# FutureSDR/FutureSDR

Hardware: NVIDIA H100
Metric: Msamples/s (higher is better)
Workload: dtype f32

## Files before the change

### futuresdr_b200/csrc/common.cuh

```cuda
#pragma once

#include <cuda_runtime.h>

#include <atomic>
#include <cstdarg>
#include <cstdint>
#include <cstdio>
#include <cstring>
#include <memory>
#include <mutex>
#include <string>
#include <vector>

#include "b200sdr.h"

struct b2s_ctx {
    int device = 0;
    cudaStream_t stream = nullptr;
    bool owns_stream = false;
    cudaStream_t s_h2d = nullptr, s_d2h = nullptr;
    int sm_count = 0;
    size_t smem_optin = 0;
    std::atomic<uint64_t> launches{0};
    std::string err;
    void *ws_dev = nullptr;
    size_t ws_bytes = 0;
    cudaEvent_t hev[16] = {};
    bool hev_ready = false;
    std::mutex host_mu;
    unsigned *d_status = nullptr;
    uint64_t flag_ops = 0;
    std::atomic<uint64_t> bytes_held{0};
};

struct PerDeviceOnce {
    std::atomic<uint64_t> mask{0};
    bool need(int dev) const { return ((mask.load(std::memory_order_acquire) >> (dev & 63)) & 1ull) == 0; }
    void done(int dev) { mask.fetch_or(1ull << (dev & 63), std::memory_order_release); }
};

#ifdef __CUDACC__
__device__ __forceinline__ void mac(float &acc, float x, float t) { acc = fmaf(x, t, acc); }
__device__ __forceinline__ void mac(float2 &acc, float2 x, float t) {
    acc.x = fmaf(x.x, t, acc.x);
    acc.y = fmaf(x.y, t, acc.y);
}
__device__ __forceinline__ void mac(float2 &acc, float2 x, float2 t) {
    acc.x = fmaf(x.x, t.x, acc.x);
    acc.x = fmaf(-x.y, t.y, acc.x);
    acc.y = fmaf(x.x, t.y, acc.y);
    acc.y = fmaf(x.y, t.x, acc.y);
}

template <typename S> __device__ __forceinline__ S zero_of();
template <> __device__ __forceinline__ float zero_of<float>() { return 0.0f; }
template <> __device__ __forceinline__ float2 zero_of<float2>() { return make_float2(0.f, 0.f); }

namespace cp_async {
__device__ __forceinline__ void ca4(float *dst_smem, const float *src) {
    const unsigned d = (unsigned)__cvta_generic_to_shared(dst_smem);
    asm volatile("cp.async.ca.shared.global [%0], [%1], 4;" ::"r"(d), "l"(src) : "memory");
}
__device__ __forceinline__ void ca4(float *dst_smem, const float *src, bool valid) {
    const unsigned d = (unsigned)__cvta_generic_to_shared(dst_smem);
    asm volatile("cp.async.ca.shared.global [%0], [%1], 4, %2;" ::"r"(d), "l"(src), "r"(valid ? 4 : 0) : "memory");
}
__device__ __forceinline__ void cg16(void *dst_smem, const void *src) {
    const unsigned d = (unsigned)__cvta_generic_to_shared(dst_smem);
    asm volatile("cp.async.cg.shared.global [%0], [%1], 16;" ::"r"(d), "l"(src) : "memory");
}
__device__ __forceinline__ void cg16(void *dst_smem, const void *src, bool valid) {
    const unsigned d = (unsigned)__cvta_generic_to_shared(dst_smem);
    asm volatile("cp.async.cg.shared.global [%0], [%1], 16, %2;" ::"r"(d), "l"(src), "r"(valid ? 16 : 0) : "memory");
}
__device__ __forceinline__ void commit() { asm volatile("cp.async.commit_group;" ::: "memory"); }
template <int N> __device__ __forceinline__ void wait() { asm volatile("cp.async.wait_group %0;" ::"n"(N) : "memory"); }
}
#endif

extern thread_local std::string g_b2s_last_error;

int32_t b2s_fail(b2s_ctx *ctx, int32_t code, const char *fmt, ...);

#define B2S_CUDA(ctx, expr)                                                                   \
    do {                                                                                      \
        cudaError_t e__ = (expr);                                                             \
        if (e__ != cudaSuccess)                                                               \
            return b2s_fail((ctx), B2S_ECUDA, "%s failed: %s (%s:%d)", #expr,                 \
                            cudaGetErrorString(e__), __FILE__, __LINE__);                     \
    } while (0)

#define B2S_CHECK_LAUNCH(ctx)                                                                 \
    do {                                                                                      \
        (ctx)->launches.fetch_add(1, std::memory_order_relaxed);                              \
        B2S_CUDA((ctx), cudaGetLastError());                                                  \
    } while (0)

struct DeviceGuard {
    int prev = -1;
    explicit DeviceGuard(int dev) {
        cudaGetDevice(&prev);
        if (prev != dev) cudaSetDevice(dev);
        else prev = -1;
    }
    ~DeviceGuard() {
        if (prev >= 0) cudaSetDevice(prev);
    }
};

#define B2S_TRY(expr)                                                                         \
    do {                                                                                      \
        const int32_t rc__ = (expr);                                                          \
        if (rc__ != B2S_OK) return rc__;                                                      \
    } while (0)

template <auto K>
int32_t smem_optin(b2s_ctx *ctx, size_t bytes, int threads = 0, int *resident = nullptr) {
    static PerDeviceOnce optin;
    static std::atomic<int> ctas[64];
    if (bytes > 48 * 1024 && optin.need(ctx->device)) {
        B2S_CUDA(ctx, cudaFuncSetAttribute(K, cudaFuncAttributeMaxDynamicSharedMemorySize, (int)bytes));
        optin.done(ctx->device);
    }
    if (resident) {
        std::atomic<int> &n = ctas[ctx->device & 63];
        int r = n.load(std::memory_order_relaxed);
        if (!r) {
            if (cudaOccupancyMaxActiveBlocksPerMultiprocessor(&r, K, threads, bytes) != cudaSuccess || r < 1) { cudaGetLastError(); r = 1; }
            n.store(r, std::memory_order_relaxed);
        }
        *resident = r;
    }
    return B2S_OK;
}

enum class Mem { Device, Pinned };

template <typename T, Mem M = Mem::Device>
class Buf {
  public:
    Buf() = default;
    Buf(Buf &&o) noexcept { swap(o); }
    Buf &operator=(Buf &&o) noexcept {
        Buf(std::move(o)).swap(*this);
        return *this;
    }
    ~Buf() { reset(); }

    T *get() const { return p_; }
    size_t size() const { return n_; }
    explicit operator bool() const { return p_ != nullptr; }

    void reset() {
        if (!ctx_) return;
        if (M == Mem::Device) cudaFree(p_);
        else cudaFreeHost(p_);
        ctx_->bytes_held -= n_ * sizeof(T);
        ctx_ = nullptr; p_ = nullptr; n_ = 0;
    }
    int32_t alloc(b2s_ctx *ctx, size_t n, const char *what) {
        reset();
        void *p = nullptr;
        const cudaError_t e = M == Mem::Device ? cudaMalloc(&p, n * sizeof(T))
                                               : cudaHostAlloc(&p, n * sizeof(T), cudaHostAllocDefault);
        if (e != cudaSuccess) {
            cudaGetLastError();
            return b2s_fail(ctx, B2S_ENOMEM, "%s: %zu bytes: %s", what, n * sizeof(T), cudaGetErrorString(e));
        }
        ctx_ = ctx; p_ = static_cast<T *>(p); n_ = n;
        ctx->bytes_held += n * sizeof(T);
        return B2S_OK;
    }
    int32_t upload(b2s_ctx *ctx, const T *host, size_t n, const char *what) {
        B2S_TRY(alloc(ctx, n, what));
        B2S_CUDA(ctx, cudaMemcpyAsync(p_, host, n * sizeof(T), cudaMemcpyHostToDevice, ctx->stream));
        return B2S_OK;
    }
    int32_t reserve(b2s_ctx *ctx, size_t n, const char *what) {
        if (n_ >= n) return B2S_OK;
        B2S_CUDA(ctx, cudaStreamSynchronize(ctx->stream));
        return alloc(ctx, n, what);
    }

  private:
    void swap(Buf &o) noexcept {
        std::swap(ctx_, o.ctx_); std::swap(p_, o.p_); std::swap(n_, o.n_);
    }
    b2s_ctx *ctx_ = nullptr;
    T *p_ = nullptr;
    size_t n_ = 0;
};

template <typename P> struct PlanDeleter {
    void operator()(P *p) const {
        if (!p) return;
        DeviceGuard g(p->ctx->device);
        cudaStreamSynchronize(p->ctx->stream);
        delete p;
    }
};
template <typename P> using PlanPtr = std::unique_ptr<P, PlanDeleter<P>>;

void nvtx_push(const char *name);
void nvtx_pop();
struct NvtxRange { explicit NvtxRange(const char *n) { nvtx_push(n); } ~NvtxRange() { nvtx_pop(); } };
int32_t peer_flag_set_launch(b2s_ctx *ctx, unsigned *flag, unsigned value, cudaStream_t st);
int32_t peer_flag_wait_launch(b2s_ctx *ctx, const unsigned *flag, unsigned value, cudaStream_t st);

static inline size_t sat_sub(size_t a, size_t b) { return a > b ? a - b : 0; }
static inline size_t ceil_div(size_t a, size_t b) { return (a + b - 1) / b; }
static inline size_t round_up(size_t a, size_t b) { return ceil_div(a, b) * b; }

static inline bool overlap(const void *p, size_t pb, const void *q, size_t qb) {
    const uintptr_t a = (uintptr_t)p, b = (uintptr_t)q;
    return pb && qb && a < b + qb && b < a + pb;
}
static inline bool bad_alias(const void *out, size_t ob, size_t oi, const void *in, size_t ib, size_t ii) {
    if (!overlap(out, ob, in, ib)) return false;
    return !(out == in && oi == ii);
}
static inline bool word_aligned(const void *p) { return ((uintptr_t)p & 3) == 0; }

static inline size_t kind_in_bytes(b2s_kind k) { return k == B2S_F32_F32 ? 4 : 8; }
static inline size_t kind_tap_floats(b2s_kind k) { return k == B2S_C32_C32 ? 2 : 1; }
```

### futuresdr_b200/csrc/pfbarb.cu

```cuda
#include <cmath>
#include <cstdlib>

#include "pfb_common.cuh"

namespace {
constexpr int kSB = 32;
constexpr int kPaThreads = 256;
constexpr int kDescCap = 4096;
constexpr int kPaSmemMax = 3 * kDescCap * 4 + 2 * 64 * 1024;

struct SubRec {
    uint32_t out0;
    float tau;
    float mu;
    uint32_t base_flag;
};
}

struct b2s_pfbarb {
    b2s_ctx *ctx = nullptr;
    size_t num_filters = 0, T = 0, ntaps = 0;
    float rate = 1.f, delay = 1.f;
    Buf<float2> d_arms;
    PfbWindows win;
    float tau = 0.f, bf = 0.f, mu = 0.f;
    size_t base_index = 0;
    bool boundary = false;
    bool periodic = false;
    uint64_t lambda = 0, out_per_period = 0, gpos = 0;
    std::vector<SubRec> tab;
    Buf<SubRec> d_tab;
    Buf<SubRec, Mem::Pinned> h_recs;
    Buf<SubRec> d_recs;
};

namespace {

__host__ __device__ __forceinline__ uint32_t pfb_arm_index(float bf) {
    const float f = floorf(bf);
    return f > 0.f ? (f < 4294967296.f ? (uint32_t)f : 0xffffffffu) : 0u;
}

inline size_t pfbarb_per_sample_max(float rate, size_t num_filters) {
    if (rate <= (float)num_filters) return (size_t)std::ceil(rate) + 1;
    return (size_t)std::ceil((double)rate * (1.0 + 1.0 / (double)num_filters)) + 2;
}

__device__ __forceinline__ float2 pfb_x(const float2 *__restrict__ hist, const float2 *__restrict__ in, int L,
                                        long long idx) {
    return idx < L ? hist[idx] : __ldg(in + (idx - L));
}

struct PaParams {
    const float2 *in, *hist;
    float2 *out;
    const float2 *arms;
    const SubRec *recs;
    long long n_in, nsub, nout;
    int sub_per_cta, N, T, sb_len;
    float delay;
    int arms_in_smem, tile_in_smem, tile_cap;
    int periodic;
    unsigned long long lambda, out_per_period, R, g0, lsb_first;
    long long O_g0;
};

struct SubStart { float tau, mu; uint32_t base_flag; long long s_beg, s_end, o_start; };

__device__ __forceinline__ SubStart pfb_sub_start(const PaParams &P, long long i) {
    SubStart r;
    if (P.periodic) {
        const unsigned long long lsb = P.lsb_first + (unsigned long long)i;
        const unsigned long long k = lsb / P.R, j = lsb - k * P.R;
        const SubRec rec = P.recs[j];
        const unsigned long long gs = k * P.lambda + j * (unsigned long long)P.sb_len;
        const unsigned long long ge = min(gs + (unsigned long long)P.sb_len, (k + 1) * P.lambda);
        r.tau = rec.tau; r.mu = rec.mu; r.base_flag = rec.base_flag;
        r.s_beg = (long long)gs - (long long)P.g0;
        r.s_end = min((long long)ge - (long long)P.g0, P.n_in);
        r.o_start = (long long)(k * P.out_per_period + rec.out0) - P.O_g0;
    } else {
        const SubRec rec = P.recs[i];
        r.tau = rec.tau; r.mu = rec.mu; r.base_flag = rec.base_flag;
        r.s_beg = i * P.sb_len;
        r.s_end = min(r.s_beg + P.sb_len, P.n_in);
        r.o_start = rec.out0;
    }
    return r;
}

__global__ void __launch_bounds__(kPaThreads) pfb_kernel(const PaParams P) {
    extern __shared__ __align__(16) unsigned char psm[];
    uint32_t *d_s1 = reinterpret_cast<uint32_t *>(psm);
    uint32_t *d_b0 = d_s1 + kDescCap;
    float *d_mu = reinterpret_cast<float *>(d_b0 + kDescCap);
    float2 *s_x = reinterpret_cast<float2 *>(d_mu + kDescCap);
    float2 *s_arms = s_x + (P.tile_in_smem ? P.tile_cap : 0);
    const int N = P.N, T = P.T;

    const long long sb0 = (long long)blockIdx.x * P.sub_per_cta;
    const long long sb1 = min(sb0 + P.sub_per_cta, P.nsub);
    const SubStart first = pfb_sub_start(P, sb0);
    const long long o_first = max(first.o_start, 0ll);
    const long long o_end = sb1 == P.nsub ? P.nout : pfb_sub_start(P, sb1).o_start;
    const long long s_lo = max(first.s_beg, 0ll);
    const long long s_hi = pfb_sub_start(P, sb1 - 1).s_end;
    const int TS = P.arms_in_smem ? (T | 1) : T;
    float *s_tap = reinterpret_cast<float *>(s_arms);
    if (P.arms_in_smem)
        for (int j = threadIdx.x; j < N * T; j += kPaThreads) s_tap[(j / T) * TS + (j % T)] = P.arms[j].x;
    if (P.tile_in_smem) {
        const int cnt = (int)(s_hi - s_lo) + T;
        for (int j = threadIdx.x; j < cnt; j += kPaThreads) s_x[j] = pfb_x(P.hist, P.in, T, s_lo + j);
    }

    for (long long sb = sb0 + threadIdx.x; sb < sb1; sb += kPaThreads) {
        const SubStart r = pfb_sub_start(P, sb);
        float tau = r.tau, mu = r.mu;
        uint32_t base = r.base_flag & 0x7fffffffu;
        bool boundary = (r.base_flag >> 31) != 0;
        long long o = r.o_start - o_first;
        const float fN = (float)N, delay = P.delay;
        for (long long s = r.s_beg; s < r.s_end; s++) {
            while (base < (uint32_t)N) {
                if (boundary) {
                    if (s >= 0) { d_s1[o] = (uint32_t)(s + 1 - s_lo) | 0x80000000u; d_b0[o] = (uint32_t)(N - 1); d_mu[o] = mu; }
                    o++;
                    tau = __fadd_rn(tau, delay);
                    const float bf = __fmul_rn(tau, fN);
                    base = pfb_arm_index(bf);
                    mu = __fsub_rn(bf, (float)base);
                    boundary = false;
                } else if (base == (uint32_t)(N - 1)) {
                    boundary = true;
                    base = (uint32_t)N;
                } else {
                    if (s >= 0) { d_s1[o] = (uint32_t)(s + 1 - s_lo); d_b0[o] = base; d_mu[o] = mu; }
                    o++;
                    tau = __fadd_rn(tau, delay);
                    const float bf = __fmul_rn(tau, fN);
                    base = pfb_arm_index(bf);
                    mu = __fsub_rn(bf, (float)base);
                }
            }
            tau = __fsub_rn(tau, 1.0f);
            base -= (uint32_t)N;
        }
    }
    __syncthreads();

    const float2 *A = P.arms;
    const uint32_t cnt = (uint32_t)(o_end - o_first);
    for (uint32_t o = threadIdx.x; o < cnt; o += kPaThreads) {
        const uint32_t w = d_s1[o];
        const bool boundary = (w >> 31) != 0;
        const int s1 = (int)(w & 0x7fffffffu);
        const uint32_t b0 = d_b0[o];
        const float mu = d_mu[o];
        const float2 *pr = A + (size_t)b0 * T;
        float2 y0 = make_float2(0.f, 0.f), y1 = make_float2(0.f, 0.f);
        if (P.tile_in_smem && P.arms_in_smem) {
            const float *t0 = s_tap + b0 * TS, *t1 = s_tap + (b0 + 1 == (uint32_t)N ? 0u : b0 + 1) * TS;
            const float2 *xb = s_x + s1;
            if (!boundary) {
#pragma unroll 4
                for (int j = 0; j < T; j++) {
                    const float2 v = xb[j];
                    const float ta = t0[j], tb = t1[j];
                    y0.x = fmaf(v.x, ta, y0.x); y0.y = fmaf(v.y, ta, y0.y);
                    y1.x = fmaf(v.x, tb, y1.x); y1.y = fmaf(v.y, tb, y1.y);
                }
            } else {
                const float2 *xa = xb - 1;
                for (int j = 0; j < T; j++) {
                    const float2 va = xa[j], vb = xb[j];
                    const float ta = t0[j], tb = t1[j];
                    y0.x = fmaf(va.x, ta, y0.x); y0.y = fmaf(va.y, ta, y0.y);
                    y1.x = fmaf(vb.x, tb, y1.x); y1.y = fmaf(vb.y, tb, y1.y);
                }
            }
        } else if (P.tile_in_smem) {
            const float2 *xb = s_x + s1;
            if (!boundary) {
#pragma unroll 4
                for (int j = 0; j < T; j++) {
                    const float2 v = xb[j], t = pr[j];
                    y0.x = fmaf(v.x, t.x, y0.x); y0.y = fmaf(v.y, t.x, y0.y);
                    y1.x = fmaf(v.x, t.y, y1.x); y1.y = fmaf(v.y, t.y, y1.y);
                }
            } else {
                const float2 *xa = xb - 1;
                for (int j = 0; j < T; j++) {
                    const float2 va = xa[j], vb = xb[j], t = pr[j];
                    y0.x = fmaf(va.x, t.x, y0.x); y0.y = fmaf(va.y, t.x, y0.y);
                    y1.x = fmaf(vb.x, t.y, y1.x); y1.y = fmaf(vb.y, t.y, y1.y);
                }
            }
        } else {
            const int s0 = boundary ? s1 - 1 : s1;
            for (int j = 0; j < T; j++) {
                const float2 va = pfb_x(P.hist, P.in, T, s_lo + s0 + j), vb = pfb_x(P.hist, P.in, T, s_lo + s1 + j);
                const float2 t = pr[j];
                y0.x = fmaf(va.x, t.x, y0.x); y0.y = fmaf(va.y, t.x, y0.y);
                y1.x = fmaf(vb.x, t.y, y1.x); y1.y = fmaf(vb.y, t.y, y1.y);
            }
        }
        const float a = __fsub_rn(1.0f, mu);
        float2 r;
        r.x = __fadd_rn(__fmul_rn(a, y0.x), __fmul_rn(mu, y1.x));
        r.y = __fadd_rn(__fmul_rn(a, y0.y), __fmul_rn(mu, y1.y));
        P.out[(size_t)o_first + o] = r;
    }
}

struct Timing {
    float tau = 0.f, mu = 0.f;
    uint32_t base = 0;
    bool boundary = false;
    bool operator==(const Timing &o) const { return tau == o.tau && mu == o.mu && base == o.base && boundary == o.boundary; }
    inline uint32_t step(uint32_t N, float fN, float delay) {
        uint32_t o = 0;
        while (base < N) {
            if (boundary) {
                o++;
                tau = tau + delay; const float bf = tau * fN; base = pfb_arm_index(bf); mu = bf - (float)base;
                boundary = false;
            } else if (base == N - 1) {
                boundary = true;
                base = N;
            } else {
                o++;
                tau = tau + delay; const float bf = tau * fN; base = pfb_arm_index(bf); mu = bf - (float)base;
            }
        }
        tau = tau - 1.0f;
        base -= N;
        return o;
    }
    SubRec rec(uint32_t out0) const { return SubRec{out0, tau, mu, base | (boundary ? 0x80000000u : 0u)}; }
};

constexpr int kPerSB = 8;
constexpr uint64_t kMaxPeriod = 1ull << 25;

bool build_periodic_schedule(b2s_pfbarb *p) {
    const uint32_t N = (uint32_t)p->num_filters;
    const float fN = (float)N, delay = p->delay;
    Timing tort, hare;
    uint64_t power = 1, lam = 1;
    hare.step(N, fN, delay);
    while (!(tort == hare)) {
        if (power == lam) {
            if (power > kMaxPeriod) return false;
            tort = hare; power *= 2; lam = 0;
        }
        hare.step(N, fN, delay);
        lam++;
    }
    if (lam > kMaxPeriod) return false;
    const uint64_t R = ceil_div((size_t)lam, (size_t)kPerSB);
    std::vector<SubRec> tab(R);
    Timing t;
    uint64_t o = 0;
    for (uint64_t s = 0; s < lam; s++) {
        if ((s % kPerSB) == 0) tab[s / kPerSB] = t.rec((uint32_t)o);
        o += t.step(N, fN, delay);
        if (o >= (1ull << 32)) return false;
    }
    if (!(t == Timing())) return false;
    p->tab.swap(tab);
    p->lambda = lam; p->out_per_period = o;
    return true;
}

uint64_t outputs_before(const b2s_pfbarb *p, uint64_t c) {
    if (c >= p->lambda) return p->out_per_period + outputs_before(p, c - p->lambda);
    const uint64_t j = c / kPerSB;
    const SubRec &r = p->tab[j];
    Timing t;
    t.tau = r.tau; t.mu = r.mu; t.base = r.base_flag & 0x7fffffffu; t.boundary = (r.base_flag >> 31) != 0;
    uint64_t o = r.out0;
    const uint32_t N = (uint32_t)p->num_filters;
    for (uint64_t s = j * kPerSB; s < c; s++) o += t.step(N, (float)N, p->delay);
    return o;
}

}

extern "C" {

int32_t b2s_pfbarb_period(float rate, size_t num_filters, uint64_t *period_items, uint64_t *outputs_per_period) {
    if (!(rate > 0.f) || num_filters == 0 || !period_items || !outputs_per_period)
        return b2s_fail(nullptr, B2S_EINVAL, "b2s_pfbarb_period: bad argument");
    b2s_pfbarb tmp;
    tmp.num_filters = num_filters; tmp.rate = rate; tmp.delay = 1.0f / rate;
    const bool ok = build_periodic_schedule(&tmp);
    *period_items = ok ? tmp.lambda : 0;
    *outputs_per_period = ok ? tmp.out_per_period : 0;
    return B2S_OK;
}

int32_t b2s_pfbarb_plan_c32(b2s_ctx *ctx, const float *taps, size_t ntaps, size_t num_filters, float rate,
                            b2s_pfbarb **out) {
    if (!ctx || !out || !taps) return b2s_fail(ctx, B2S_EINVAL, "b2s_pfbarb_plan_c32: NULL argument");
    *out = nullptr;
    if (!(rate > 0.f)) return b2s_fail(ctx, B2S_EINVAL, "PfbArbResampler: resampling rate must be greater than zero");
    if (num_filters == 0) return b2s_fail(ctx, B2S_EINVAL, "PfbArbResampler: number of filter banks must be greater than zero");
    if (ntaps < num_filters) return b2s_fail(ctx, B2S_EINVAL, "PfbArbResampler: prototype filter length must be at least num_filters");
    if (num_filters > (1u << 20) || rate > 126.f || pfbarb_per_sample_max(rate, num_filters) * kSB > (size_t)kDescCap)
        return b2s_fail(ctx, B2S_EUNSUPPORTED, "PfbArbResampler: rate %f too large for %zu arms (a sample may produce more outputs than one CTA holds)", (double)rate, num_filters);
    DeviceGuard g(ctx->device);
    PlanPtr<b2s_pfbarb> p(new b2s_pfbarb());
    p->ctx = ctx; p->num_filters = num_filters; p->ntaps = ntaps; p->rate = rate;
    p->delay = 1.0f / rate;
    std::vector<float> arms;
    const size_t T = pfb_partition(taps, ntaps, num_filters, arms);
    p->T = T;
    std::vector<float2> pairs(num_filters * T);
    for (size_t b = 0; b < num_filters; b++)
        for (size_t j = 0; j < T; j++)
            pairs[b * T + j] = make_float2(arms[b * T + T - 1 - j], arms[((b + 1) % num_filters) * T + T - 1 - j]);
    B2S_TRY(p->d_arms.upload(ctx, pairs.data(), pairs.size(), "pfbarb arms"));
    B2S_TRY(p->win.init(ctx, 1, (int)T, false, "pfbarb history"));
    p->periodic = getenv("B2S_PFBARB_NO_PERIODIC") ? false : build_periodic_schedule(p.get());
    if (p->periodic) B2S_TRY(p->d_tab.upload(ctx, p->tab.data(), p->tab.size(), "pfbarb schedule table"));
    B2S_TRY(smem_optin<pfb_kernel>(ctx, kPaSmemMax));
    B2S_CUDA(ctx, cudaStreamSynchronize(ctx->stream));
    B2S_TRY(b2s_pfbarb_reset(p.get()));
    *out = p.release();
    return B2S_OK;
}

void b2s_pfbarb_destroy(b2s_pfbarb *p) { PlanDeleter<b2s_pfbarb>()(p); }

int32_t b2s_pfbarb_reset(b2s_pfbarb *p) {
    if (!p) return b2s_fail(nullptr, B2S_EINVAL, "pfbarb is NULL");
    DeviceGuard g(p->ctx->device);
    p->tau = 0.f; p->bf = 0.f; p->mu = 0.f; p->base_index = 0; p->boundary = false;
    p->gpos = 0;
    return p->win.reset(p->ctx);
}

int32_t b2s_pfbarb_exec(b2s_pfbarb *p, const void *d_in, size_t n_in, void *d_out, size_t n_out_cap,
                        size_t *consumed, size_t *produced, int32_t *call_again) {
    if (!p || !consumed || !produced || !call_again) return b2s_fail(p ? p->ctx : nullptr, B2S_EINVAL, "b2s_pfbarb_exec: NULL argument");
    b2s_ctx *ctx = p->ctx;
    *consumed = 0; *produced = 0; *call_again = 0;
    DeviceGuard g(ctx->device);
    const int T = (int)p->T;
    const float2 *in = (const float2 *)d_in;
    if (!p->win.full()) {
        const size_t c = std::min(p->win.missing(), n_in);
        B2S_TRY(p->win.push(ctx, in, c));
        *consumed = c;
        if (n_in - c > 0) *call_again = 1;
        return B2S_OK;
    }
    const size_t cap = (size_t)((float)n_out_cap / p->rate);
    const size_t n = std::min(n_in, cap);
    if (n == 0) return B2S_OK;
    if (!d_in || !d_out) return b2s_fail(ctx, B2S_EINVAL, "b2s_pfbarb_exec: NULL buffer");
    if (n >= (1ull << 31)) return b2s_fail(ctx, B2S_EUNSUPPORTED, "b2s_pfbarb_exec: more than 2^31 items per call");
    NvtxRange nvtx("b2s_pfbarb_exec");
    PaParams P{};
    P.in = in; P.hist = p->win.hist.get(); P.out = (float2 *)d_out; P.arms = p->d_arms.get();
    P.n_in = (long long)n; P.N = (int)p->num_filters; P.T = T; P.delay = p->delay;
    size_t nout;
    Timing after;
    if (p->periodic) {
        const uint64_t g0 = p->gpos, g1 = g0 + n, lam = p->lambda, R = p->tab.size();
        const uint64_t O0 = outputs_before(p, g0);
        const uint64_t O1 = (g1 / lam) * p->out_per_period + outputs_before(p, g1 % lam);
        nout = (size_t)(O1 - O0);
        if (nout > n_out_cap)
            return b2s_fail(ctx, B2S_ESTATE, "pfbarb: schedule produces %zu > capacity %zu (the reference would overrun its slice)", nout, n_out_cap);
        const uint64_t lsb_first = g0 / kPerSB;
        const uint64_t gl = g1 - 1, lsb_last = (gl / lam) * R + (gl % lam) / kPerSB;
        P.periodic = 1; P.recs = p->d_tab.get(); P.sb_len = kPerSB;
        P.lambda = lam; P.out_per_period = p->out_per_period; P.R = R; P.g0 = g0; P.lsb_first = lsb_first;
        P.O_g0 = (long long)O0;
        P.nsub = (long long)(lsb_last - lsb_first + 1);
    } else {
        const size_t nsub = ceil_div(n, (size_t)kSB);
        B2S_CUDA(ctx, cudaStreamSynchronize(ctx->stream));
        if (std::min(p->d_recs.size(), p->h_recs.size()) < nsub + 1) {
            const size_t want = (nsub + 1) * 5 / 4 + 16;
            B2S_TRY(p->d_recs.reserve(ctx, want, "pfbarb records"));
            B2S_TRY(p->h_recs.reserve(ctx, want, "pfbarb pinned records"));
        }
        Timing t;
        t.tau = p->tau; t.mu = p->mu; t.base = (uint32_t)p->base_index; t.boundary = p->boundary;
        const uint32_t N = (uint32_t)p->num_filters;
        uint64_t o = 0;
        for (size_t s = 0; s < n; s++) {
            if ((s % kSB) == 0) p->h_recs.get()[s / kSB] = t.rec((uint32_t)o);
            o += t.step(N, (float)N, p->delay);
        }
        p->h_recs.get()[nsub] = t.rec((uint32_t)o);
        nout = (size_t)o;
        if (nout > n_out_cap || o >= (1ull << 32))
            return b2s_fail(ctx, B2S_ESTATE, "pfbarb: schedule produces %zu > capacity %zu (the reference would overrun its slice)", nout, n_out_cap);
        after = t;
        B2S_CUDA(ctx, cudaMemcpyAsync(p->d_recs.get(), p->h_recs.get(), (nsub + 1) * sizeof(SubRec), cudaMemcpyHostToDevice, ctx->stream));
        P.periodic = 0; P.recs = p->d_recs.get(); P.sb_len = kSB; P.nsub = (long long)nsub;
    }
    P.nout = (long long)nout;
    const size_t per_sample_max = pfbarb_per_sample_max(p->rate, p->num_filters);
    size_t sub_per_cta = kDescCap / (per_sample_max * P.sb_len);
    if (sub_per_cta == 0) return b2s_fail(ctx, B2S_EUNSUPPORTED, "pfbarb: rate %f too high for the descriptor tile", (double)p->rate);
    sub_per_cta = std::min<size_t>(sub_per_cta, kPaThreads);
    P.sub_per_cta = (int)sub_per_cta;
    const unsigned grid = (unsigned)ceil_div((size_t)P.nsub, sub_per_cta);
    const size_t tile_items = sub_per_cta * P.sb_len + p->T + 2;
    P.tile_in_smem = tile_items * sizeof(float2) <= 64 * 1024;
    P.tile_cap = (int)tile_items;
    const size_t arms_smem_bytes = p->num_filters * (p->T | 1) * sizeof(float);
    P.arms_in_smem = arms_smem_bytes <= 64 * 1024;
    const size_t smem = 3 * kDescCap * sizeof(uint32_t) + (P.tile_in_smem ? tile_items * sizeof(float2) : 0) +
                        (P.arms_in_smem ? arms_smem_bytes : 0);
    pfb_kernel<<<grid, kPaThreads, smem, ctx->stream>>>(P);
    B2S_CHECK_LAUNCH(ctx);
    B2S_TRY(p->win.slide(ctx, in, 0, (long long)n));
    if (p->periodic) p->gpos = (p->gpos + n) % p->lambda;
    else { p->tau = after.tau; p->mu = after.mu; p->base_index = after.base; p->boundary = after.boundary; }
    *consumed = n; *produced = nout;
    return B2S_OK;
}

}
```

Measured before the change: 168,900.

## Add one-pass persistent PFB arbitrary resampler kernel with double-buffered cp.async tiles

Adds a new persistent one-pass kernel, templated on tap width, for small filters (T<=32 with arms fitting in shared memory). Each thread replays the timing for an 8-sample chunk and computes the outputs directly from register windows, which removes the separate descriptor-building pass and its shared-memory descriptor arrays. Input tiles are double-buffered with cp.async, using padded slots to avoid bank conflicts, and outputs are staged in shared memory so global stores are coalesced. It also adds a 32-bit fast path for the periodic-schedule division and debug knockout flags. The cost is extra replay work per chunk, register pressure from the templated windows, and more complexity, while the old kernel remains as a fallback.

```diff
diff --git a/futuresdr_b200/csrc/common.cuh b/futuresdr_b200/csrc/common.cuh
--- a/futuresdr_b200/csrc/common.cuh
+++ b/futuresdr_b200/csrc/common.cuh
@@ -65,6 +65,10 @@
     const unsigned d = (unsigned)__cvta_generic_to_shared(dst_smem);
     asm volatile("cp.async.ca.shared.global [%0], [%1], 4, %2;" ::"r"(d), "l"(src), "r"(valid ? 4 : 0) : "memory");
 }
+__device__ __forceinline__ void ca8(void *dst_smem, const void *src) {
+    const unsigned d = (unsigned)__cvta_generic_to_shared(dst_smem);
+    asm volatile("cp.async.ca.shared.global [%0], [%1], 8;" ::"r"(d), "l"(src) : "memory");
+}
 __device__ __forceinline__ void cg16(void *dst_smem, const void *src) {
     const unsigned d = (unsigned)__cvta_generic_to_shared(dst_smem);
     asm volatile("cp.async.cg.shared.global [%0], [%1], 16;" ::"r"(d), "l"(src) : "memory");
diff --git a/futuresdr_b200/csrc/pfbarb.cu b/futuresdr_b200/csrc/pfbarb.cu
--- a/futuresdr_b200/csrc/pfbarb.cu
+++ b/futuresdr_b200/csrc/pfbarb.cu
@@ -8,6 +8,11 @@
 constexpr int kPaThreads = 256;
 constexpr int kDescCap = 4096;
 constexpr int kPaSmemMax = 3 * kDescCap * 4 + 2 * 64 * 1024;
+constexpr int kChunk = 8;
+constexpr int kSpan = kPaThreads * kChunk;
+constexpr int kOutStageMax = 6144;
+constexpr int kArmsSmemMax = 64 * 1024;
+constexpr int kKoStage = 1, kKoReplay = 2, kKoDot = 4, kKoStore = 8, kForceDesc = 16;
 
 struct SubRec {
     uint32_t out0;
@@ -27,6 +32,8 @@
     size_t base_index = 0;
     bool boundary = false;
     bool periodic = false;
+    int flags = 0;
+    int resident = 0;
     uint64_t lambda = 0, out_per_period = 0, gpos = 0;
     std::vector<SubRec> tab;
     Buf<SubRec> d_tab;
@@ -60,6 +67,7 @@
     int sub_per_cta, N, T, sb_len;
     float delay;
     int arms_in_smem, tile_in_smem, tile_cap;
+    int flags, stage_cap;
     int periodic;
     unsigned long long lambda, out_per_period, R, g0, lsb_first;
     long long O_g0;
@@ -71,7 +79,8 @@
     SubStart r;
     if (P.periodic) {
         const unsigned long long lsb = P.lsb_first + (unsigned long long)i;
-        const unsigned long long k = lsb / P.R, j = lsb - k * P.R;
+        const unsigned long long k = (lsb >> 32) == 0 && (P.R >> 32) == 0 ? (unsigned)lsb / (unsigned)P.R : lsb / P.R;
+        const unsigned long long j = lsb - k * P.R;
         const SubRec rec = P.recs[j];
         const unsigned long long gs = k * P.lambda + j * (unsigned long long)P.sb_len;
         const unsigned long long ge = min(gs + (unsigned long long)P.sb_len, (k + 1) * P.lambda);
@@ -89,7 +98,7 @@
     return r;
 }
 
-__global__ void __launch_bounds__(kPaThreads) pfb_kernel(const PaParams P) {
+__global__ void __launch_bounds__(kPaThreads) pfb_desc_kernel(const PaParams P) {
     extern __shared__ __align__(16) unsigned char psm[];
     uint32_t *d_s1 = reinterpret_cast<uint32_t *>(psm);
     uint32_t *d_b0 = d_s1 + kDescCap;
@@ -109,12 +118,16 @@
     float *s_tap = reinterpret_cast<float *>(s_arms);
     if (P.arms_in_smem)
         for (int j = threadIdx.x; j < N * T; j += kPaThreads) s_tap[(j / T) * TS + (j % T)] = P.arms[j].x;
-    if (P.tile_in_smem) {
+    if (P.tile_in_smem && !(P.flags & kKoStage)) {
         const int cnt = (int)(s_hi - s_lo) + T;
         for (int j = threadIdx.x; j < cnt; j += kPaThreads) s_x[j] = pfb_x(P.hist, P.in, T, s_lo + j);
     }
-
-    for (long long sb = sb0 + threadIdx.x; sb < sb1; sb += kPaThreads) {
+    if (P.flags & kKoReplay)
+        for (long long o = threadIdx.x; o < o_end - o_first; o += kPaThreads) {
+            d_s1[o] = (uint32_t)min(o * 4 / 3, s_hi - s_lo - 1) + 1; d_b0[o] = (uint32_t)(o % N); d_mu[o] = 0.5f;
+        }
+
+    for (long long sb = sb0 + threadIdx.x; sb < (P.flags & kKoReplay ? sb0 : sb1); sb += kPaThreads) {
         const SubStart r = pfb_sub_start(P, sb);
         float tau = r.tau, mu = r.mu;
         uint32_t base = r.base_flag & 0x7fffffffu;
@@ -159,7 +172,9 @@
         const float mu = d_mu[o];
         const float2 *pr = A + (size_t)b0 * T;
         float2 y0 = make_float2(0.f, 0.f), y1 = make_float2(0.f, 0.f);
-        if (P.tile_in_smem && P.arms_in_smem) {
+        if (P.flags & kKoDot) {
+            y0 = y1 = make_float2((float)s1, mu);
+        } else if (P.tile_in_smem && P.arms_in_smem) {
             const float *t0 = s_tap + b0 * TS, *t1 = s_tap + (b0 + 1 == (uint32_t)N ? 0u : b0 + 1) * TS;
             const float2 *xb = s_x + s1;
             if (!boundary) {
@@ -209,8 +224,164 @@
         float2 r;
         r.x = __fadd_rn(__fmul_rn(a, y0.x), __fmul_rn(mu, y1.x));
         r.y = __fadd_rn(__fmul_rn(a, y0.y), __fmul_rn(mu, y1.y));
-        P.out[(size_t)o_first + o] = r;
-    }
+        if (!(P.flags & kKoStore)) P.out[(size_t)o_first + o] = r;
+    }
+}
+
+__host__ __device__ constexpr int pfb_slot(int k) { return k + (k >> 3); }
+template <int TW> constexpr int kTileSlots = pfb_slot(kSpan + TW + kChunk) + 1;
+
+struct SpanHdr { long long o_first, o_end, s_lo, s_hi; };
+
+template <int TW>
+__global__ void __launch_bounds__(kPaThreads) pfb_kernel(const PaParams P) {
+    extern __shared__ __align__(16) unsigned char psm[];
+    __shared__ SpanHdr hdr[2];
+    float2 *s_out = reinterpret_cast<float2 *>(psm);
+    float2 *s_tiles = s_out + P.stage_cap;
+    float2 *s_tap = s_tiles + 2 * kTileSlots<TW>;
+    const int N = P.N, T = P.T;
+    const uint32_t uN = (uint32_t)N;
+    const int cps = P.sb_len / kChunk;
+    const long long rec_per_cta = kPaThreads / cps;
+    const long long nspan = (P.nsub + rec_per_cta - 1) / rec_per_cta;
+
+    auto header = [&](long long span, SpanHdr &h) {
+        const long long sb0 = span * rec_per_cta, sb1 = min(sb0 + rec_per_cta, P.nsub);
+        if (threadIdx.x == 0) {
+            const SubStart f = pfb_sub_start(P, sb0);
+            h.o_first = max(f.o_start, 0ll); h.s_lo = max(f.s_beg, 0ll);
+        } else if (threadIdx.x == 32) {
+            h.o_end = sb1 == P.nsub ? P.nout : pfb_sub_start(P, sb1).o_start;
+        } else if (threadIdx.x == 64) {
+            h.s_hi = pfb_sub_start(P, sb1 - 1).s_end;
+        }
+    };
+    auto stage = [&](const SpanHdr &h, float2 *s_x) {
+        if (!(P.flags & kKoStage)) {
+            const int cnt = (int)(h.s_hi - h.s_lo) + T;
+            for (int j = threadIdx.x; j < cnt; j += kPaThreads) {
+                const long long idx = h.s_lo + j;
+                cp_async::ca8(s_x + pfb_slot(j), idx < T ? P.hist + idx : P.in + (idx - T));
+            }
+        }
+        cp_async::commit();
+    };
+
+    long long span = blockIdx.x;
+    if (span >= nspan) return;
+    header(span, hdr[0]);
+    for (int j = threadIdx.x; j < N * T; j += kPaThreads) s_tap[(j / T) * (T + 1) + (j % T)] = P.arms[j];
+    __syncthreads();
+    stage(hdr[0], s_tiles);
+    for (int buf = 0; span < nspan; span += gridDim.x, buf ^= 1) {
+        const long long next = span + gridDim.x;
+        if (next < nspan) header(next, hdr[buf ^ 1]);
+        const long long sb0 = span * rec_per_cta, sb1 = min(sb0 + rec_per_cta, P.nsub);
+        const long long rec = sb0 + threadIdx.x / cps;
+        const SubStart r = pfb_sub_start(P, min(rec, sb1 - 1));
+        cp_async::wait<0>();
+        __syncthreads();
+        if (next < nspan) stage(hdr[buf ^ 1], s_tiles + (buf ^ 1) * kTileSlots<TW>);
+        const SpanHdr h = hdr[buf];
+        const float2 *s_x = s_tiles + buf * kTileSlots<TW>;
+        const long long o_first = h.o_first, s_lo = h.s_lo;
+        const int ocnt = (int)(h.o_end - o_first);
+        const bool staged = ocnt <= P.stage_cap;
+        if (rec < sb1) {
+            float tau = r.tau, mu = r.mu;
+            uint32_t base = r.base_flag & 0x7fffffffu;
+            bool boundary = (r.base_flag >> 31) != 0;
+            int o = (int)(r.o_start - o_first);
+            const float fN = (float)N, delay = P.delay;
+            const long long c_beg = r.s_beg + (long long)(threadIdx.x % cps) * kChunk;
+            const long long e0 = max(c_beg, 0ll), e1 = min(c_beg + kChunk, r.s_end);
+            for (long long s = r.s_beg; s < e0; s++) {
+                while (base < uN) {
+                    if (!boundary && base == uN - 1) { boundary = true; base = uN; continue; }
+                    o++;
+                    tau = __fadd_rn(tau, delay);
+                    const float bf = __fmul_rn(tau, fN);
+                    base = pfb_arm_index(bf);
+                    mu = __fsub_rn(bf, (float)base);
+                    boundary = false;
+                }
+                tau = __fsub_rn(tau, 1.0f);
+                base -= uN;
+            }
+            const int len = (int)(e1 - e0);
+            const bool ko_replay = (P.flags & kKoReplay) != 0;
+            int o_lim = ocnt;
+            if (ko_replay && rec + 1 < sb1) o_lim = min(o_lim, (int)(pfb_sub_start(P, rec + 1).o_start - o_first));
+            if (len > 0) {
+                float2 w[kChunk + TW];
+                const int rb = (int)(e0 - s_lo);
+    #pragma unroll
+                for (int k = 0; k < kChunk + TW; k++) w[k] = s_x[pfb_slot(rb + k)];
+    #pragma unroll
+                for (int i = 0; i < kChunk; i++) {
+                    if (i < len) {
+                        if (ko_replay) { base = o < o_lim ? (uint32_t)(i * 5) % uN : uN; boundary = false; mu = 0.5f; }
+                        while (base < uN) {
+                            if (!boundary && base == uN - 1) { boundary = true; base = uN; continue; }
+                            const uint32_t b0 = boundary ? uN - 1 : base;
+                            const float2 *tpair = s_tap + b0 * (T + 1);
+                            float2 y0 = make_float2(0.f, 0.f), y1 = make_float2(0.f, 0.f);
+                            if (P.flags & kKoDot) {
+                                y0 = y1 = w[i + 1];
+                            } else {
+    #pragma unroll
+                                for (int j = 0; j < TW; j++) {
+                                    if (j < T) {
+                                        const float2 va = boundary ? w[i + j] : w[i + 1 + j], vb = w[i + 1 + j];
+                                        const float2 tp = tpair[j];
+                                        const float ta = tp.x, tb = tp.y;
+                                        y0.x = fmaf(va.x, ta, y0.x); y0.y = fmaf(va.y, ta, y0.y);
+                                        y1.x = fmaf(vb.x, tb, y1.x); y1.y = fmaf(vb.y, tb, y1.y);
+                                    }
+                                }
+                            }
+                            const float a = __fsub_rn(1.0f, mu);
+                            float2 y;
+                            y.x = __fadd_rn(__fmul_rn(a, y0.x), __fmul_rn(mu, y1.x));
+                            y.y = __fadd_rn(__fmul_rn(a, y0.y), __fmul_rn(mu, y1.y));
+                            if (!(P.flags & kKoStore)) {
+                                if (staged) s_out[o] = y;
+                                else P.out[o_first + o] = y;
+                            }
+                            o++;
+                            if (ko_replay) { base = uN; break; }
+                            tau = __fadd_rn(tau, delay);
+                            const float bf = __fmul_rn(tau, fN);
+                            base = pfb_arm_index(bf);
+                            mu = __fsub_rn(bf, (float)base);
+                            boundary = false;
+                        }
+                        tau = __fsub_rn(tau, 1.0f);
+                        base -= uN;
+                    }
+                }
+            }
+        }
+        __syncthreads();
+        if (staged && !(P.flags & kKoStore))
+            for (int k = threadIdx.x; k < ocnt; k += kPaThreads) P.out[o_first + k] = s_out[k];
+    }
+}
+
+inline size_t pfbarb_one_pass_arms(const b2s_pfbarb *p) {
+    return p->num_filters * (p->T + 1) * sizeof(float2);
+}
+inline bool pfbarb_one_pass(const b2s_pfbarb *p) {
+    return p->T <= 32 && pfbarb_one_pass_arms(p) <= (size_t)kArmsSmemMax && !(p->flags & kForceDesc);
+}
+inline int pfbarb_tw(size_t T) { return T <= 8 ? 8 : T <= 16 ? 16 : 32; }
+inline int pfbarb_stage_cap(float rate) {
+    const double want = std::ceil((double)kSpan * rate) + 256;
+    return want >= kOutStageMax ? kOutStageMax : (int)ceil_div((size_t)want, (size_t)32) * 32;
+}
+inline size_t pfbarb_one_pass_smem(int TW, int stage_cap, size_t arms_bytes) {
+    return (size_t)stage_cap * sizeof(float2) + (size_t)2 * (pfb_slot(kSpan + TW + kChunk) + 1) * sizeof(float2) + arms_bytes;
 }
 
 struct Timing {
@@ -324,7 +495,11 @@
     B2S_TRY(p->win.init(ctx, 1, (int)T, false, "pfbarb history"));
     p->periodic = getenv("B2S_PFBARB_NO_PERIODIC") ? false : build_periodic_schedule(p.get());
     if (p->periodic) B2S_TRY(p->d_tab.upload(ctx, p->tab.data(), p->tab.size(), "pfbarb schedule table"));
-    B2S_TRY(smem_optin<pfb_kernel>(ctx, kPaSmemMax));
+    p->flags = getenv("B2S_PFBARB_FLAGS") ? (int)strtol(getenv("B2S_PFBARB_FLAGS"), nullptr, 0) : 0;
+    B2S_TRY(smem_optin<pfb_desc_kernel>(ctx, kPaSmemMax));
+    B2S_TRY(smem_optin<pfb_kernel<8>>(ctx, pfbarb_one_pass_smem(8, kOutStageMax, kArmsSmemMax)));
+    B2S_TRY(smem_optin<pfb_kernel<16>>(ctx, pfbarb_one_pass_smem(16, kOutStageMax, kArmsSmemMax)));
+    B2S_TRY(smem_optin<pfb_kernel<32>>(ctx, pfbarb_one_pass_smem(32, kOutStageMax, kArmsSmemMax)));
     B2S_CUDA(ctx, cudaStreamSynchronize(ctx->stream));
     B2S_TRY(b2s_pfbarb_reset(p.get()));
     *out = p.release();
@@ -405,20 +580,40 @@
         P.periodic = 0; P.recs = p->d_recs.get(); P.sb_len = kSB; P.nsub = (long long)nsub;
     }
     P.nout = (long long)nout;
-    const size_t per_sample_max = pfbarb_per_sample_max(p->rate, p->num_filters);
-    size_t sub_per_cta = kDescCap / (per_sample_max * P.sb_len);
-    if (sub_per_cta == 0) return b2s_fail(ctx, B2S_EUNSUPPORTED, "pfbarb: rate %f too high for the descriptor tile", (double)p->rate);
-    sub_per_cta = std::min<size_t>(sub_per_cta, kPaThreads);
-    P.sub_per_cta = (int)sub_per_cta;
-    const unsigned grid = (unsigned)ceil_div((size_t)P.nsub, sub_per_cta);
-    const size_t tile_items = sub_per_cta * P.sb_len + p->T + 2;
-    P.tile_in_smem = tile_items * sizeof(float2) <= 64 * 1024;
-    P.tile_cap = (int)tile_items;
-    const size_t arms_smem_bytes = p->num_filters * (p->T | 1) * sizeof(float);
-    P.arms_in_smem = arms_smem_bytes <= 64 * 1024;
-    const size_t smem = 3 * kDescCap * sizeof(uint32_t) + (P.tile_in_smem ? tile_items * sizeof(float2) : 0) +
-                        (P.arms_in_smem ? arms_smem_bytes : 0);
-    pfb_kernel<<<grid, kPaThreads, smem, ctx->stream>>>(P);
+    P.flags = p->flags;
+    if (pfbarb_one_pass(p)) {
+        P.sub_per_cta = kSpan / P.sb_len;
+        P.stage_cap = pfbarb_stage_cap(p->rate);
+        const int TW = pfbarb_tw(p->T);
+        const size_t smem = pfbarb_one_pass_smem(TW, P.stage_cap, pfbarb_one_pass_arms(p));
+        if (!p->resident) {
+            const cudaError_t e = TW == 8 ? cudaOccupancyMaxActiveBlocksPerMultiprocessor(&p->resident, pfb_kernel<8>, kPaThreads, smem)
+                                : TW == 16 ? cudaOccupancyMaxActiveBlocksPerMultiprocessor(&p->resident, pfb_kernel<16>, kPaThreads, smem)
+                                : cudaOccupancyMaxActiveBlocksPerMultiprocessor(&p->resident, pfb_kernel<32>, kPaThreads, smem);
+            B2S_CUDA(ctx, e);
+            p->resident = std::max(p->resident, 1);
+        }
+        const unsigned grid = (unsigned)std::min<size_t>(ceil_div((size_t)P.nsub, (size_t)P.sub_per_cta),
+                                                         (size_t)ctx->sm_count * (size_t)p->resident);
+        if (TW == 8) pfb_kernel<8><<<grid, kPaThreads, smem, ctx->stream>>>(P);
+        else if (TW == 16) pfb_kernel<16><<<grid, kPaThreads, smem, ctx->stream>>>(P);
+        else pfb_kernel<32><<<grid, kPaThreads, smem, ctx->stream>>>(P);
+    } else {
+        const size_t per_sample_max = pfbarb_per_sample_max(p->rate, p->num_filters);
+        size_t sub_per_cta = kDescCap / (per_sample_max * P.sb_len);
+        if (sub_per_cta == 0) return b2s_fail(ctx, B2S_EUNSUPPORTED, "pfbarb: rate %f too high for the descriptor tile", (double)p->rate);
+        sub_per_cta = std::min<size_t>(sub_per_cta, kPaThreads);
+        P.sub_per_cta = (int)sub_per_cta;
+        const unsigned grid = (unsigned)ceil_div((size_t)P.nsub, sub_per_cta);
+        const size_t tile_items = sub_per_cta * P.sb_len + p->T + 2;
+        P.tile_in_smem = tile_items * sizeof(float2) <= 64 * 1024;
+        P.tile_cap = (int)tile_items;
+        const size_t arms_smem_bytes = p->num_filters * (p->T | 1) * sizeof(float);
+        P.arms_in_smem = arms_smem_bytes <= kArmsSmemMax;
+        const size_t smem = 3 * kDescCap * sizeof(uint32_t) + (P.tile_in_smem ? tile_items * sizeof(float2) : 0) +
+                            (P.arms_in_smem ? arms_smem_bytes : 0);
+        pfb_desc_kernel<<<grid, kPaThreads, smem, ctx->stream>>>(P);
+    }
     B2S_CHECK_LAUNCH(ctx);
     B2S_TRY(p->win.slide(ctx, in, 0, (long long)n));
     if (p->periodic) p->gpos = (p->gpos + n) % p->lambda;
```

After: 168,400 (median of 6 runs). About the same (-0.3%).

## Tune pfbarb tiling for occupancy, async-copy input tile, specialize T=16 dot

Applied to the files above, without the earlier changes.

Picks the sub-blocks per CTA and the descriptor capacity at plan time by querying occupancy, sizing shared memory to what is actually needed instead of a fixed 4096-entry descriptor area. Loads the arms and input tile with cp.async (16-byte copies for aligned pairs) so the copies overlap the schedule-descriptor generation. It also computes the four block-boundary lookups in parallel across lanes and broadcasts them with shuffles, uses 32-bit index math, and adds a fully unrolled dot product for T=16. The risks are edge cases in the alignment and tail handling of the tile load, and the assumption that the periodic index fits in 32 bits.

```diff
diff --git a/futuresdr_b200/csrc/pfbarb.cu b/futuresdr_b200/csrc/pfbarb.cu
--- a/futuresdr_b200/csrc/pfbarb.cu
+++ b/futuresdr_b200/csrc/pfbarb.cu
@@ -30,6 +30,8 @@
     uint64_t lambda = 0, out_per_period = 0, gpos = 0;
     std::vector<SubRec> tab;
     Buf<SubRec> d_tab;
+    int sub_per_cta = 0, tile_in_smem = 0, tile_cap = 0, arms_in_smem = 0, desc_cap = 0;
+    size_t smem = 0;
     Buf<SubRec, Mem::Pinned> h_recs;
     Buf<SubRec> d_recs;
 };
@@ -59,7 +61,7 @@
     long long n_in, nsub, nout;
     int sub_per_cta, N, T, sb_len;
     float delay;
-    int arms_in_smem, tile_in_smem, tile_cap;
+    int arms_in_smem, tile_in_smem, tile_cap, desc_cap;
     int periodic;
     unsigned long long lambda, out_per_period, R, g0, lsb_first;
     long long O_g0;
@@ -70,8 +72,8 @@
 __device__ __forceinline__ SubStart pfb_sub_start(const PaParams &P, long long i) {
     SubStart r;
     if (P.periodic) {
-        const unsigned long long lsb = P.lsb_first + (unsigned long long)i;
-        const unsigned long long k = lsb / P.R, j = lsb - k * P.R;
+        const uint32_t lsb = (uint32_t)(P.lsb_first + (unsigned long long)i), R = (uint32_t)P.R;
+        const unsigned long long k = lsb / R, j = lsb - (uint32_t)k * R;
         const SubRec rec = P.recs[j];
         const unsigned long long gs = k * P.lambda + j * (unsigned long long)P.sb_len;
         const unsigned long long ge = min(gs + (unsigned long long)P.sb_len, (k + 1) * P.lambda);
@@ -89,42 +91,87 @@
     return r;
 }
 
+template <int TT>
+__device__ __forceinline__ void pfb_dot_smem(const float2 *xb, bool boundary, const float *t0, const float *t1, int T,
+                                             float2 &y0, float2 &y1) {
+    const int n = TT ? TT : T;
+    if (!boundary) {
+#pragma unroll(TT ? TT : 4)
+        for (int j = 0; j < n; j++) {
+            const float2 v = xb[j];
+            const float ta = t0[j], tb = t1[j];
+            y0.x = fmaf(v.x, ta, y0.x); y0.y = fmaf(v.y, ta, y0.y);
+            y1.x = fmaf(v.x, tb, y1.x); y1.y = fmaf(v.y, tb, y1.y);
+        }
+    } else {
+        const float2 *xa = xb - 1;
+#pragma unroll(TT ? TT : 4)
+        for (int j = 0; j < n; j++) {
+            const float2 va = xa[j], vb = xb[j];
+            const float ta = t0[j], tb = t1[j];
+            y0.x = fmaf(va.x, ta, y0.x); y0.y = fmaf(va.y, ta, y0.y);
+            y1.x = fmaf(vb.x, tb, y1.x); y1.y = fmaf(vb.y, tb, y1.y);
+        }
+    }
+}
+
 __global__ void __launch_bounds__(kPaThreads) pfb_kernel(const PaParams P) {
     extern __shared__ __align__(16) unsigned char psm[];
-    uint32_t *d_s1 = reinterpret_cast<uint32_t *>(psm);
-    uint32_t *d_b0 = d_s1 + kDescCap;
-    float *d_mu = reinterpret_cast<float *>(d_b0 + kDescCap);
-    float2 *s_x = reinterpret_cast<float2 *>(d_mu + kDescCap);
-    float2 *s_arms = s_x + (P.tile_in_smem ? P.tile_cap : 0);
+    float2 *s_x = reinterpret_cast<float2 *>(psm);
+    float *s_tap = reinterpret_cast<float *>(s_x + (P.tile_in_smem ? P.tile_cap : 0));
+    uint32_t *d_s1 = reinterpret_cast<uint32_t *>(s_tap + (P.arms_in_smem ? P.N * (P.T | 1) : 0));
+    uint32_t *d_b0 = d_s1 + P.desc_cap;
+    float *d_mu = reinterpret_cast<float *>(d_b0 + P.desc_cap);
     const int N = P.N, T = P.T;
 
     const long long sb0 = (long long)blockIdx.x * P.sub_per_cta;
     const long long sb1 = min(sb0 + P.sub_per_cta, P.nsub);
-    const SubStart first = pfb_sub_start(P, sb0);
-    const long long o_first = max(first.o_start, 0ll);
-    const long long o_end = sb1 == P.nsub ? P.nout : pfb_sub_start(P, sb1).o_start;
-    const long long s_lo = max(first.s_beg, 0ll);
-    const long long s_hi = pfb_sub_start(P, sb1 - 1).s_end;
+    long long mine;
+    {
+        const int l = threadIdx.x & 31;
+        const SubStart r = pfb_sub_start(P, l == 2 ? sb1 : l == 3 ? sb1 - 1 : sb0);
+        mine = l == 0 ? r.o_start : l == 1 ? r.s_beg : l == 2 ? (sb1 == P.nsub ? P.nout : r.o_start) : r.s_end;
+    }
+    const long long o_first = max(__shfl_sync(0xffffffffu, mine, 0), 0ll);
+    const long long s_lo = max(__shfl_sync(0xffffffffu, mine, 1), 0ll);
+    const long long o_end = __shfl_sync(0xffffffffu, mine, 2);
+    const long long s_hi = __shfl_sync(0xffffffffu, mine, 3);
     const int TS = P.arms_in_smem ? (T | 1) : T;
-    float *s_tap = reinterpret_cast<float *>(s_arms);
     if (P.arms_in_smem)
-        for (int j = threadIdx.x; j < N * T; j += kPaThreads) s_tap[(j / T) * TS + (j % T)] = P.arms[j].x;
+        for (int j = threadIdx.x; j < N * T; j += kPaThreads) cp_async::ca4(s_tap + (j / T) * TS + (j % T), &P.arms[j].x);
+    const float2 *xs = s_x;
     if (P.tile_in_smem) {
         const int cnt = (int)(s_hi - s_lo) + T;
-        for (int j = threadIdx.x; j < cnt; j += kPaThreads) s_x[j] = pfb_x(P.hist, P.in, T, s_lo + j);
-    }
+        const long long in8 = (long long)(reinterpret_cast<uintptr_t>(P.in) / sizeof(float2));
+        float2 *dst = s_x + ((in8 + s_lo + T) & 1);
+        xs = dst;
+        const int nh = (int)max(0ll, min((long long)cnt, T - s_lo));
+        for (int k = threadIdx.x; k < nh; k += kPaThreads) dst[k] = P.hist[s_lo + k];
+        int k0 = nh, m = cnt - nh;
+        const float2 *src = P.in + (s_lo + nh - T);
+        if (((in8 + s_lo + nh - T) & 1) && m > 0) {
+            if (threadIdx.x == 0) { cp_async::ca4(&dst[k0].x, &src->x); cp_async::ca4(&dst[k0].y, &src->y); }
+            k0++; m--; src++;
+        }
+        for (int q = threadIdx.x; q < m / 2; q += kPaThreads) cp_async::cg16(dst + k0 + 2 * q, src + 2 * q);
+        if ((m & 1) && threadIdx.x == kPaThreads - 1) {
+            cp_async::ca4(&dst[k0 + m - 1].x, &src[m - 1].x); cp_async::ca4(&dst[k0 + m - 1].y, &src[m - 1].y);
+        }
+    }
+    cp_async::commit();
 
     for (long long sb = sb0 + threadIdx.x; sb < sb1; sb += kPaThreads) {
         const SubStart r = pfb_sub_start(P, sb);
         float tau = r.tau, mu = r.mu;
         uint32_t base = r.base_flag & 0x7fffffffu;
         bool boundary = (r.base_flag >> 31) != 0;
-        long long o = r.o_start - o_first;
+        int o = (int)(r.o_start - o_first);
         const float fN = (float)N, delay = P.delay;
-        for (long long s = r.s_beg; s < r.s_end; s++) {
+        const int slo = (int)s_lo, s_end = (int)r.s_end;
+        for (int s = (int)r.s_beg; s < s_end; s++) {
             while (base < (uint32_t)N) {
                 if (boundary) {
-                    if (s >= 0) { d_s1[o] = (uint32_t)(s + 1 - s_lo) | 0x80000000u; d_b0[o] = (uint32_t)(N - 1); d_mu[o] = mu; }
+                    if (s >= 0) { d_s1[o] = (uint32_t)(s + 1 - slo) | 0x80000000u; d_b0[o] = (uint32_t)(N - 1); d_mu[o] = mu; }
                     o++;
                     tau = __fadd_rn(tau, delay);
                     const float bf = __fmul_rn(tau, fN);
@@ -135,7 +182,7 @@
                     boundary = true;
                     base = (uint32_t)N;
                 } else {
-                    if (s >= 0) { d_s1[o] = (uint32_t)(s + 1 - s_lo); d_b0[o] = base; d_mu[o] = mu; }
+                    if (s >= 0) { d_s1[o] = (uint32_t)(s + 1 - slo); d_b0[o] = base; d_mu[o] = mu; }
                     o++;
                     tau = __fadd_rn(tau, delay);
                     const float bf = __fmul_rn(tau, fN);
@@ -147,6 +194,7 @@
             base -= (uint32_t)N;
         }
     }
+    cp_async::wait<0>();
     __syncthreads();
 
     const float2 *A = P.arms;
@@ -161,26 +209,10 @@
         float2 y0 = make_float2(0.f, 0.f), y1 = make_float2(0.f, 0.f);
         if (P.tile_in_smem && P.arms_in_smem) {
             const float *t0 = s_tap + b0 * TS, *t1 = s_tap + (b0 + 1 == (uint32_t)N ? 0u : b0 + 1) * TS;
-            const float2 *xb = s_x + s1;
-            if (!boundary) {
-#pragma unroll 4
-                for (int j = 0; j < T; j++) {
-                    const float2 v = xb[j];
-                    const float ta = t0[j], tb = t1[j];
-                    y0.x = fmaf(v.x, ta, y0.x); y0.y = fmaf(v.y, ta, y0.y);
-                    y1.x = fmaf(v.x, tb, y1.x); y1.y = fmaf(v.y, tb, y1.y);
-                }
-            } else {
-                const float2 *xa = xb - 1;
-                for (int j = 0; j < T; j++) {
-                    const float2 va = xa[j], vb = xb[j];
-                    const float ta = t0[j], tb = t1[j];
-                    y0.x = fmaf(va.x, ta, y0.x); y0.y = fmaf(va.y, ta, y0.y);
-                    y1.x = fmaf(vb.x, tb, y1.x); y1.y = fmaf(vb.y, tb, y1.y);
-                }
-            }
+            if (T == 16) pfb_dot_smem<16>(xs + s1, boundary, t0, t1, T, y0, y1);
+            else pfb_dot_smem<0>(xs + s1, boundary, t0, t1, T, y0, y1);
         } else if (P.tile_in_smem) {
-            const float2 *xb = s_x + s1;
+            const float2 *xb = xs + s1;
             if (!boundary) {
 #pragma unroll 4
                 for (int j = 0; j < T; j++) {
@@ -283,6 +315,29 @@
     const uint32_t N = (uint32_t)p->num_filters;
     for (uint64_t s = j * kPerSB; s < c; s++) o += t.step(N, (float)N, p->delay);
     return o;
+}
+
+int32_t pfbarb_tiling(b2s_pfbarb *p) {
+    const size_t psm = pfbarb_per_sample_max(p->rate, p->num_filters), sb_len = p->periodic ? kPerSB : kSB;
+    const size_t arms_bytes = p->num_filters * (p->T | 1) * sizeof(float);
+    p->arms_in_smem = arms_bytes <= 64 * 1024;
+    int best = 0;
+    for (size_t sub = std::min<size_t>(kDescCap / (psm * sb_len), kPaThreads); sub >= 1; sub /= 2) {
+        const size_t tile_items = sub * sb_len + p->T + 2;
+        const int tile_in_smem = tile_items * sizeof(float2) <= 64 * 1024;
+        const size_t desc_cap = sub * sb_len * psm;
+        const size_t smem = (tile_in_smem ? tile_items * sizeof(float2) : 0) + (p->arms_in_smem ? arms_bytes : 0) +
+                            3 * desc_cap * sizeof(uint32_t);
+        int ctas = 0;
+        B2S_CUDA(p->ctx, cudaOccupancyMaxActiveBlocksPerMultiprocessor(&ctas, pfb_kernel, kPaThreads, smem));
+        if (ctas > best) {
+            best = ctas;
+            p->sub_per_cta = (int)sub; p->tile_in_smem = tile_in_smem; p->tile_cap = (int)tile_items;
+            p->desc_cap = (int)desc_cap; p->smem = smem;
+        }
+    }
+    if (best == 0) return b2s_fail(p->ctx, B2S_EUNSUPPORTED, "pfbarb: no CTA of the resampler fits an SM");
+    return B2S_OK;
 }
 
 }
@@ -325,6 +380,7 @@
     p->periodic = getenv("B2S_PFBARB_NO_PERIODIC") ? false : build_periodic_schedule(p.get());
     if (p->periodic) B2S_TRY(p->d_tab.upload(ctx, p->tab.data(), p->tab.size(), "pfbarb schedule table"));
     B2S_TRY(smem_optin<pfb_kernel>(ctx, kPaSmemMax));
+    B2S_TRY(pfbarb_tiling(p.get()));
     B2S_CUDA(ctx, cudaStreamSynchronize(ctx->stream));
     B2S_TRY(b2s_pfbarb_reset(p.get()));
     *out = p.release();
@@ -405,20 +461,10 @@
         P.periodic = 0; P.recs = p->d_recs.get(); P.sb_len = kSB; P.nsub = (long long)nsub;
     }
     P.nout = (long long)nout;
-    const size_t per_sample_max = pfbarb_per_sample_max(p->rate, p->num_filters);
-    size_t sub_per_cta = kDescCap / (per_sample_max * P.sb_len);
-    if (sub_per_cta == 0) return b2s_fail(ctx, B2S_EUNSUPPORTED, "pfbarb: rate %f too high for the descriptor tile", (double)p->rate);
-    sub_per_cta = std::min<size_t>(sub_per_cta, kPaThreads);
-    P.sub_per_cta = (int)sub_per_cta;
-    const unsigned grid = (unsigned)ceil_div((size_t)P.nsub, sub_per_cta);
-    const size_t tile_items = sub_per_cta * P.sb_len + p->T + 2;
-    P.tile_in_smem = tile_items * sizeof(float2) <= 64 * 1024;
-    P.tile_cap = (int)tile_items;
-    const size_t arms_smem_bytes = p->num_filters * (p->T | 1) * sizeof(float);
-    P.arms_in_smem = arms_smem_bytes <= 64 * 1024;
-    const size_t smem = 3 * kDescCap * sizeof(uint32_t) + (P.tile_in_smem ? tile_items * sizeof(float2) : 0) +
-                        (P.arms_in_smem ? arms_smem_bytes : 0);
-    pfb_kernel<<<grid, kPaThreads, smem, ctx->stream>>>(P);
+    P.sub_per_cta = p->sub_per_cta; P.tile_in_smem = p->tile_in_smem; P.tile_cap = p->tile_cap;
+    P.arms_in_smem = p->arms_in_smem; P.desc_cap = p->desc_cap;
+    const unsigned grid = (unsigned)ceil_div((size_t)P.nsub, (size_t)p->sub_per_cta);
+    pfb_kernel<<<grid, kPaThreads, p->smem, ctx->stream>>>(P);
     B2S_CHECK_LAUNCH(ctx);
     B2S_TRY(p->win.slide(ctx, in, 0, (long long)n));
     if (p->periodic) p->gpos = (p->gpos + n) % p->lambda;
```

Result: no change. 171,100 before, 170,600 after, median of 6 (-0.3%).
